# ZhentaoHuang/SealD-NeRF

Measured on AMD Instinct MI355X. Metric: rendered rays/sec + sampled-points/sec, 800×800 D-NeRF jumpingjacks, higher is better.
Workload: dtype f16; 1 GPU; dnerf jumpingjacks-like 800x800 full-frame inference render, -O (fp16 field network, fp16 grid table), test sequence of 20 frames (camera orbit, one time stamp per frame, t = 0 .. 1: every frame selects its own occupancy slice, time encoding and the t == 0 canonical rule), T_thresh 1e-2, max_steps 1024, dt_gamma 0; rays=640000, field=fused, loop=device, frames_per_loop=4, rays_per_loop_on_this_gpu=2560000, frames_in_flight=4 loops of 4 frame(s) (the next starts when the newest is down to rays/2 alive), parallelism=single GPU

## Files before the change

seald-nerf_amd/csrc/raymarching.hip:

```cpp
#include <stdlib.h>

#include "sdn_common.h"
#include "sdn_internal.h"

namespace {
using sdn_int::FrameSel;

constexpr float kSqrt3 = 1.7320508075688772f;
constexpr float kRPi = 0.3183098861837907f;

__device__ __forceinline__ float signf_(float x) { return copysignf(1.0f, x); }
__device__ __forceinline__ float clampf_(float x, float lo, float hi) { return fminf(hi, fmaxf(lo, x)); }

__device__ __forceinline__ int mip_from_pos(float x, float y, float z, float max_cascade) {
    const float mx = fmaxf(fabsf(x), fmaxf(fabsf(y), fabsf(z)));
    int exponent;
    frexpf(mx, &exponent);
    return (int)fminf(max_cascade - 1, fmaxf(0.0f, (float)exponent));
}
__device__ __forceinline__ int mip_from_dt(float dt, float H, float max_cascade) {
    const float mx = (float)((double)(dt * H) * 0.5);
    int exponent;
    frexpf(mx, &exponent);
    return (int)fminf(max_cascade - 1, fmaxf(0.0f, (float)exponent));
// ... 884 lines not shown
__device__ __forceinline__ bool composite_ray(int index, uint32_t n_step, float T_thresh, const float *s, const float *c, const float *dl,
                                              float *__restrict__ rays_t, float *__restrict__ weights_sum, float *__restrict__ depth,
                                              float *__restrict__ image, float *t_out = nullptr) {
    float t = rays_t[index];
    float weight_sum = weights_sum[index], d = depth[index];
    float r = image[(size_t)index * 3], g = image[(size_t)index * 3 + 1], b = image[(size_t)index * 3 + 2];
    uint32_t step = 0;
    if (n_step == 8) {
        float sv[8], cv[24], dv[16];
        #pragma unroll
        for (int q = 0; q < 2; q++) *reinterpret_cast<float4 *>(sv + 4 * q) = *reinterpret_cast<const float4 *>(s + 4 * q);
        #pragma unroll
        for (int q = 0; q < 6; q++) *reinterpret_cast<float4 *>(cv + 4 * q) = *reinterpret_cast<const float4 *>(c + 4 * q);
        #pragma unroll
        for (int q = 0; q < 4; q++) *reinterpret_cast<float4 *>(dv + 4 * q) = *reinterpret_cast<const float4 *>(dl + 4 * q);
        bool open = true;
        #pragma unroll
        for (int k = 0; k < 8; k++) {
            if (open && dv[2 * k] == 0) open = false;
            if (open) {
                const float alpha = 1.0f - sdn_exp_cr(-sv[k] * dv[2 * k]);
                const float T = 1 - weight_sum;
                const float weight = alpha * T;
                weight_sum += weight;
                t += dv[2 * k + 1];
                d += weight * t;
                r += weight * cv[3 * k]; g += weight * cv[3 * k + 1]; b += weight * cv[3 * k + 2];
                if (T < T_thresh) open = false; else step++;
            }
        }
    } else {
        while (step < n_step) {
            if (dl[0] == 0) break;
            const float alpha = 1.0f - sdn_exp_cr(-s[0] * dl[0]);
            const float T = 1 - weight_sum;
            const float weight = alpha * T;
            weight_sum += weight;
            t += dl[1];
            d += weight * t;
            r += weight * c[0]; g += weight * c[1]; b += weight * c[2];
            if (T < T_thresh) break;
            s++; c += 3; dl += 2; step++;
        }
    }
    const bool survives = !(step < n_step);
    if (survives) rays_t[index] = t;
    if (t_out) *t_out = t;
    weights_sum[index] = weight_sum; depth[index] = d;
    image[(size_t)index * 3] = r; image[(size_t)index * 3 + 1] = g; image[(size_t)index * 3 + 2] = b;
    return survives;
}

template <bool FAST>
__global__ void __launch_bounds__(256) k_march_rays(uint32_t n_alive, uint32_t n_step, const int32_t *__restrict__ rays_alive,
                                                    const float *__restrict__ rays_t, const float *__restrict__ rays_o,
                                                    const float *__restrict__ rays_d, float bound, float dt_gamma, uint32_t max_steps,
                                                    uint32_t C, uint32_t H, const uint8_t *__restrict__ grid,
                                                    const float *__restrict__ fars, float *__restrict__ xyzs, float *__restrict__ dirs,
                                                    float *__restrict__ deltas, const float *__restrict__ noises, uint32_t M_pad,
                                                    const uint32_t *__restrict__ cull, uint32_t *__restrict__ live_idx,
                                                    uint32_t *__restrict__ live_count, const int32_t *__restrict__ state,
                                                    const int32_t *__restrict__ rays_alive_b, FrameSel fs, const float *__restrict__ jump) {
    if (state) {
        n_alive = (uint32_t)state[0];
        n_step = (uint32_t)state[1];
        if (n_alive == 0) return;
        if (state[4]) rays_alive = rays_alive_b;
        live_count += state[3];
        const uint32_t m0 = n_alive * n_step;
        M_pad = m0 + (128u - m0 % 128u);
        if (!(state[15] && state[3] == 0)) jump = nullptr;
        if (blockIdx.x * 256u >= n_alive + 128u) return;
    }
    __shared__ uint4 s_cull4[FAST ? 256 : 1];
    __shared__ unsigned long long s_fine[FAST ? kFineCacheCells : 1];
    __shared__ uint32_t s_min4[4];
    const uint32_t n = threadIdx.x + blockIdx.x * blockDim.x;
    const int index = n < n_alive ? rays_alive[n] : -1;
    const bool grouped = fs.n_frames > 1;
    const uint32_t frame = (grouped && index >= 0) ? (uint32_t)index / fs.rays_per_frame : (grouped ? kNoFrame : 0u);
    uint32_t step = 0;
    float ro[3] = {0, 0, 0}, rdv[3] = {0, 0, 1}, t_ray = 0, far_ray = 0, t_jump = 0, noise = 0;
    if (index >= 0) {
        ro[0] = rays_o[(size_t)index * 3]; ro[1] = rays_o[(size_t)index * 3 + 1]; ro[2] = rays_o[(size_t)index * 3 + 2];
        rdv[0] = rays_d[(size_t)index * 3]; rdv[1] = rays_d[(size_t)index * 3 + 1]; rdv[2] = rays_d[(size_t)index * 3 + 2];
        t_ray = rays_t[index]; far_ray = fars[index];
        if (jump) t_jump = jump[index];
        if (noises) noise = noises[n];
    }
    uint32_t fcur = grouped ? block_min_256(frame, s_min4) : 0u;
    while (fcur != kNoFrame) {
        const uint8_t *grid_f = grouped ? frame_grid_uniform(fs, fcur) : grid;
        const uint32_t *cull_f = (grouped && cull) ? cull + (size_t)fcur * fs.cull_stride : cull;
        OccCache oc;
        occ_cache_load<FAST>(cull_f, grid_f, s_cull4, s_fine, oc);
        if (index >= 0 && frame == fcur) {
            MarcherT<FAST> m;
            m.init(ro, rdv, bound, dt_gamma, max_steps, C, H, grid_f);
            float t = t_ray;
            t += m.step_size(t) * noise;
            float *tend = state ? state_tend(state) : nullptr;
            if (tend) tend += index;
            const float t_walk = jump ? t_jump : t;
            step = march_ray<FAST>(m, oc, t_walk, far_ray, n_step, xyzs + (size_t)n * n_step * 3, dirs + (size_t)n * n_step * 3,
                                   deltas + (size_t)n * n_step * 2, tend, grouped ? fs.slot_frame + (size_t)n * n_step : nullptr, frame,
                                   jump ? &t : nullptr);
        }
        if (!grouped) break;
        fcur = block_min_256((frame != kNoFrame && frame > fcur) ? frame : kNoFrame, s_min4);
    }
    if (n >= n_alive) {
        const uint32_t slot = n_alive * n_step + (n - n_alive);
        if (slot < M_pad) {
            xyzs[(size_t)slot * 3] = 0; xyzs[(size_t)slot * 3 + 1] = 0; xyzs[(size_t)slot * 3 + 2] = 0;
            dirs[(size_t)slot * 3] = 0; dirs[(size_t)slot * 3 + 1] = 0; dirs[(size_t)slot * 3 + 2] = 0;
            deltas[(size_t)slot * 2] = 0; deltas[(size_t)slot * 2 + 1] = 0;
        }
    }
    if (live_idx) live_append(step, n, n_step, live_idx, live_count);
}

__device__ __forceinline__ uint32_t loop_list_len(const int32_t *__restrict__ state) {
    return state[8] ? (uint32_t)state[8] : (uint32_t)state[0];
}

__global__ void __launch_bounds__(256) k_composite_rays(uint32_t n_alive, uint32_t n_step, float T_thresh, int32_t *__restrict__ rays_alive,
                                                        float *__restrict__ rays_t, const float *__restrict__ sigmas,
                                                        const float *__restrict__ rgbs, const float *__restrict__ deltas,
                                                        float *__restrict__ weights_sum, float *__restrict__ depth, float *__restrict__ image,
                                                        const int32_t *__restrict__ state, int32_t *__restrict__ rays_alive_b,
                                                        uint32_t *__restrict__ block_totals) {
    if (state) {
        n_alive = loop_list_len(state);
        n_step = (uint32_t)state[1];
        if (state[4]) rays_alive = rays_alive_b;
    }
    const uint32_t n = threadIdx.x + blockIdx.x * blockDim.x;
    bool survives = false;
    if (n < n_alive) {
        const int index = rays_alive[n];
        if (index >= 0) {
            survives = composite_ray(index, n_step, T_thresh, sigmas + (size_t)n * n_step, rgbs + (size_t)n * n_step * 3,
                                     deltas + (size_t)n * n_step * 2, rays_t, weights_sum, depth, image);
            if (!survives) rays_alive[n] = -1;
        }
    }
    if (block_totals) {
        __shared__ uint32_t s_cnt[4];
        const unsigned long long m = __ballot(survives);
        if ((threadIdx.x & 63u) == 0) s_cnt[threadIdx.x >> 6] = (uint32_t)__popcll(m);
        __syncthreads();
        if (threadIdx.x == 0) block_totals[blockIdx.x] = s_cnt[0] + s_cnt[1] + s_cnt[2] + s_cnt[3];
    }
}

__global__ void __launch_bounds__(kScanBlock) k_compact_count(const int32_t *__restrict__ in, uint32_t n, uint32_t *__restrict__ block_totals,
                                                              const int32_t *__restrict__ state, const int32_t *__restrict__ in_b) {
    if (state) {
        n = loop_list_len(state);
        if (state[4]) in = in_b;
        if (blockIdx.x * kScanBlock >= n) return;
    }
    __shared__ uint32_t lds[16];
    const uint32_t i = blockIdx.x * kScanBlock + threadIdx.x;
    const bool keep = i < n && in[i] >= 0;
    const unsigned long long mask = __ballot(keep);
    if ((threadIdx.x & 63u) == 0) lds[threadIdx.x >> 6] = (uint32_t)__popcll(mask);
    __syncthreads();
    if (threadIdx.x == 0) {
        uint32_t t = 0;
        for (uint32_t w = 0; w < (kScanBlock >> 6); w++) t += lds[w];
        block_totals[blockIdx.x] = t;
// ... 332 lines not shown
            if (!survives) alive[n] = -1;
        }
        const bool marches = survives && march_next;
        const bool grouped = fs.n_frames > 1;
        const uint32_t frame = (grouped && marches) ? (uint32_t)index / fs.rays_per_frame : (grouped ? kNoFrame : 0u);
        uint32_t fcur = grouped ? block_min_256(frame, s_min4) : 0u;
        while (fcur != kNoFrame) {
            const uint8_t *grid_f = grouped ? frame_grid_uniform(fs, fcur) : grid;
            const uint32_t *cull_f = (grouped && cull) ? cull + (size_t)fcur * fs.cull_stride : cull;
            OccCache oc;
            occ_cache_load<FAST>(cull_f, grid_f, s_cull4, s_fine, oc);
            if (marches && frame == fcur) {
                float *px = xyzs + (size_t)n * n_step * 3, *pd = dirs + (size_t)n * n_step * 3, *pl = deltas + (size_t)n * n_step * 2;
                MarcherT<FAST> m;
                m.init(ro, rdv, bound, dt_gamma, max_steps, C, H, grid_f);
                float *tend = state_tend(state);
                if (tend) tend += index;
                emitted = march_ray<FAST>(m, oc, t_new, far_ray, n_step, px, pd, pl, tend,
                                          grouped ? fs.slot_frame + (size_t)n * n_step : nullptr, frame);
            }
            if (!grouped) break;
            fcur = block_min_256((frame != kNoFrame && frame > fcur) ? frame : kNoFrame, s_min4);
        }
        live_append(emitted, n, n_step, live_idx, live_counts + it + 1);
    }
    const unsigned long long mask = __ballot(survives);
    if ((threadIdx.x & 63u) == 0) s_cnt[threadIdx.x >> 6] = (uint32_t)__popcll(mask);
    __syncthreads();
    if (threadIdx.x == 0) {
        const uint32_t c = s_cnt[0] + s_cnt[1] + s_cnt[2] + s_cnt[3];
        if (c) atomicAdd(state + 9, (int32_t)c);
        __threadfence();
        s_last = (atomicAdd(ticket, 1) == (int)gridDim.x - 1);
    }
    __syncthreads();
    if (!s_last || threadIdx.x != 0) return;
    __threadfence();
    *ticket = 0;
    const int32_t call = state[7];
    state[7] = call + 1;
    if (state[0] > 0) {
        trace[2 * it] = state[0];
        trace[2 * it + 1] = state[1];
        state[2] += state[1];
        state[3] = it + 1;
        int32_t n_new = atomicAdd(state + 9, 0);
        state[9] = 0;
        if (state[2] >= state[6]) n_new = 0;
        state[0] = n_new;
    }
    publish_snapshot(state, snap, call);
}

__global__ void __launch_bounds__(256) k_loop_finish(uint32_t N, const float *__restrict__ nears, const float *__restrict__ fars,
                                                     const float *__restrict__ weights_sum, const float *__restrict__ depth,
                                                     const float *__restrict__ image, float bg, float *__restrict__ image_out,
                                                     float *__restrict__ depth_out) {
    const uint32_t n = threadIdx.x + blockIdx.x * blockDim.x;
    if (n >= N) return;
    const float w = (1 - weights_sum[n]) * bg;
    image_out[(size_t)n * 3] = image[(size_t)n * 3] + w;
    image_out[(size_t)n * 3 + 1] = image[(size_t)n * 3 + 1] + w;
    image_out[(size_t)n * 3 + 2] = image[(size_t)n * 3 + 2] + w;
    depth_out[n] = fmaxf(depth[n] - nears[n], 0.0f) / (fars[n] - nears[n]);
}

struct MarchRays {
    uint32_t threads = 0;
    uint32_t n_alive = 0, n_step = 0;
    const int32_t *rays_alive = nullptr, *rays_alive_b = nullptr, *state = nullptr;
    const float *rays_t = nullptr, *rays_o = nullptr, *rays_d = nullptr, *fars = nullptr, *noises = nullptr;
    float bound = 0, dt_gamma = 0;
    uint32_t max_steps = 0, C = 0, H = 0, M_pad = 0;
    const uint8_t *grid = nullptr;
    float *xyzs = nullptr, *dirs = nullptr, *deltas = nullptr;
    const uint32_t *cull = nullptr;
    uint32_t *live_idx = nullptr, *live_count = nullptr;
    FrameSel fs;
    const float *jump = nullptr;
};
int launch_k_march_rays(const MarchRays &m, hipStream_t st) {
    const dim3 g(sdn_div_up(m.threads, 256u)), b(256);
    if (fast_config(m.bound, m.C, m.H)) {
        const uint32_t *cull = (m.cull && m.H != 128) ? nullptr : m.cull;
        hipLaunchKernelGGL(k_march_rays<true>, g, b, 0, st, m.n_alive, m.n_step, m.rays_alive, m.rays_t, m.rays_o, m.rays_d, m.bound, m.dt_gamma,
                           m.max_steps, m.C, m.H, m.grid, m.fars, m.xyzs, m.dirs, m.deltas, m.noises, m.M_pad, cull, m.live_idx, m.live_count, m.state,
                           m.rays_alive_b, m.fs, cull ? m.jump : (const float *)nullptr);
    } else {
        hipLaunchKernelGGL(k_march_rays<false>, g, b, 0, st, m.n_alive, m.n_step, m.rays_alive, m.rays_t, m.rays_o, m.rays_d, m.bound, m.dt_gamma,
                           m.max_steps, m.C, m.H, m.grid, m.fars, m.xyzs, m.dirs, m.deltas, m.noises, m.M_pad, (const uint32_t *)nullptr, m.live_idx,
                           m.live_count, m.state, m.rays_alive_b, m.fs, (const float *)nullptr);
    }
    return sdn_launch_status();
}

struct TrainScratch { uint64_t cull, sample_t; };
TrainScratch train_scratch(uint32_t N) {
    const uint64_t words = (uint64_t)N + sdn_div_up(N, kScanBlock) + 4u;
    const uint64_t head = (words * sizeof(uint32_t) + 15u) & ~(uint64_t)15u;
    const uint64_t cull_bytes = ((uint64_t)(kCullWords + 8u) * sizeof(uint32_t) + 15u) & ~(uint64_t)15u;
    return {head, head + cull_bytes};
}

}

namespace sdn_int {

int loop_begin(const SdnRenderCtx &c, void *mailbox, uint32_t frame_tag, hipStream_t st) {
    const uint32_t threads = c.N > c.n_counters ? c.N : c.n_counters;
    hipLaunchKernelGGL(k_loop_init, dim3(sdn_div_up(threads, 256u)), dim3(256), 0, st, c.N, c.max_steps, c.nears, c.alive_a, c.rays_t, c.weights_sum,
                       c.depth, c.image, c.state, c.live_counts, c.n_counters, (unsigned long long)(uintptr_t)mailbox, frame_tag, c.rays_tend);
    return sdn_launch_status();
}

int loop_cull_start(const SdnRenderCtx &c, hipStream_t st) {
    const uint32_t *cull = loop_cull(c);
    if (!cull || !c.rays_tend || c.H != 128 || !fast_config(c.bound, c.C, c.H)) return 0;
    uint32_t *block_totals = (uint32_t *)c.block_totals;
    hipLaunchKernelGGL(k_cull_start, dim3(sdn_div_up(c.N, 256u)), dim3(256), 0, st, c.N, c.rays_o, c.rays_d, c.nears, c.fars, cull, frame_sel(c), c.alive_a,
                       c.rays_tend, c.bound, c.dt_gamma, c.max_steps, c.C, c.H, jump_buffer(c), block_totals);
    const uint32_t nb = sdn_div_up(c.N, kScanBlock);
    hipLaunchKernelGGL(k_compact_scatter, dim3(nb), dim3(kScanBlock), 0, st, (const int32_t *)c.alive_a, c.N, (const uint32_t *)block_totals, c.alive_b,
                       snap_n_out(c), (const int32_t *)nullptr, (const int32_t *)nullptr, (int32_t *)nullptr, 4u);
    hipLaunchKernelGGL(k_cull_advance, dim3(1), dim3(64), 0, st, c.state, (const int32_t *)snap_n_out(c), c.trace);
    return sdn_launch_status();
}

static int march(const SdnRenderCtx &c, uint32_t bound_alive, const float *jump, hipStream_t st) {
    MarchRays m;
    m.threads = bound_alive + 128u;
    m.rays_alive = c.alive_a; m.rays_alive_b = c.alive_b; m.rays_t = c.rays_t; m.rays_o = c.rays_o; m.rays_d = c.rays_d;
    m.bound = c.bound; m.dt_gamma = c.dt_gamma; m.max_steps = c.max_steps; m.C = c.C; m.H = c.H; m.grid = c.bitfield; m.fars = c.fars;
    m.xyzs = c.xyzs; m.dirs = c.dirs; m.deltas = c.deltas; m.cull = loop_cull(c); m.live_idx = c.live_idx; m.live_count = live_counters(c);
    m.state = c.state; m.fs = frame_sel(c); m.jump = jump;
    return launch_k_march_rays(m, st);
}

int loop_march(const SdnRenderCtx &c, uint32_t bound_alive, hipStream_t st) { return march(c, bound_alive, jump_buffer(c), st); }

int loop_composite_compact(const SdnRenderCtx &c, uint32_t bound_alive, hipStream_t st, bool freeze) {
    const dim3 g(sdn_div_up(bound_alive, 256u)), b(256);
    uint32_t *block_totals = (uint32_t *)c.block_totals;
    int32_t *snap = snap_ring(c);
    hipLaunchKernelGGL(k_composite_rays, g, b, 0, st, 0u, 0u, c.T_thresh, c.alive_a, c.rays_t, c.sigmas, c.rgbs, c.deltas, c.weights_sum, c.depth, c.image,
                       (const int32_t *)c.state, c.alive_b, block_totals);
    if (bound_alive > 65536u) {
        static_assert(kScanBlock == 1024, "the compositing kernel's 256-ray survivor counts are summed four to a scatter block");
        const uint32_t nb = sdn_div_up(bound_alive, kScanBlock);
        hipLaunchKernelGGL(k_compact_scatter, dim3(nb), dim3(kScanBlock), 0, st, (const int32_t *)c.alive_a, 0u, (const uint32_t *)block_totals,
                           c.alive_b, snap_n_out(c), (const int32_t *)c.state, (const int32_t *)c.alive_b, c.alive_a, 4u);
        hipLaunchKernelGGL(k_loop_advance, dim3(1), dim3(64), 0, st, c.state, (const int32_t *)snap_n_out(c), c.trace, snap, freeze ? 1 : 0);
        return sdn_launch_status();
    }
    hipLaunchKernelGGL(k_scatter_advance, g, b, 0, st, c.alive_a, c.alive_b, (const uint32_t *)block_totals, c.state, c.n_out, c.trace, snap, freeze ? 1 : 0);
    return sdn_launch_status();
}

int loop_steady_begin(const SdnRenderCtx &c, uint32_t bound_alive, hipStream_t st, bool frozen_already) {
    if (!frozen_already) hipLaunchKernelGGL(k_steady_begin, dim3(1), dim3(64), 0, st, c.state);
    return march(c, bound_alive, nullptr, st);
}

int loop_composite_march(const SdnRenderCtx &c, uint32_t bound_list, hipStream_t st) {
    const dim3 g(sdn_div_up(bound_list, 256u)), b(256);
    const FrameSel fs = frame_sel(c);
    int32_t *snap = snap_ring(c);
    if (fast_config(c.bound, c.C, c.H)) {
        const uint32_t *cull = loop_cull(c);
        if (cull && c.H != 128) cull = nullptr;
        hipLaunchKernelGGL(k_composite_march<true>, g, b, 0, st, c.T_thresh, c.alive_a, c.alive_b, c.rays_t, c.rays_o, c.rays_d, c.bound, c.dt_gamma,
                           c.max_steps, c.C, c.H, c.bitfield, c.fars, c.sigmas, c.rgbs, c.xyzs, c.dirs, c.deltas, c.weights_sum, c.depth, c.image, cull,
                           c.live_idx, live_counters(c), c.state, c.n_out, c.trace, snap, fs);
    } else {
        hipLaunchKernelGGL(k_composite_march<false>, g, b, 0, st, c.T_thresh, c.alive_a, c.alive_b, c.rays_t, c.rays_o, c.rays_d, c.bound, c.dt_gamma,
                           c.max_steps, c.C, c.H, c.bitfield, c.fars, c.sigmas, c.rgbs, c.xyzs, c.dirs, c.deltas, c.weights_sum, c.depth, c.image,
                           (const uint32_t *)nullptr, c.live_idx, live_counters(c), c.state, c.n_out, c.trace, snap, fs);
    }
    return sdn_launch_status();
}

int loop_finish(const SdnRenderCtx &c, float bg, float *image_out, float *depth_out, hipStream_t st) {
    hipLaunchKernelGGL(k_loop_finish, dim3(sdn_div_up(c.N, 256u)), dim3(256), 0, st, c.N, c.nears, c.fars, c.weights_sum, c.depth, c.image, bg, image_out,
                       depth_out);
    return sdn_launch_status();
}

int build_cull(const uint8_t *bitfield, uint32_t *cull_bits, hipStream_t st, bool with_image) {
    hipLaunchKernelGGL(k_cull_meta_init, dim3(1), dim3(64), 0, st, cull_bits, 1u, 0u);
    hipLaunchKernelGGL(k_build_cull_grid, dim3(kCullRes * kCullRes * kCullRes / 256), dim3(256), 0, st, bitfield, cull_bits, FrameSel());
    if (with_image) hipLaunchKernelGGL(k_build_fine_image, dim3(kFineCacheCells / 256), dim3(256), 0, st, bitfield, cull_bits, FrameSel());
    return sdn_launch_status();
}

struct CullCopy { const uint32_t *src[SDN_MAX_GROUP_FRAMES]; };
__global__ void __launch_bounds__(256) k_copy_cull_grids(CullCopy srcs, uint32_t *__restrict__ dst, uint32_t words, uint32_t stride) {
    const uint32_t i = blockIdx.x * blockDim.x + threadIdx.x;
    if (i < words) dst[(size_t)blockIdx.y * stride + i] = srcs.src[blockIdx.y][i];
}

int copy_cull(const void *const *prebuilt, uint32_t n_frames, uint32_t *cull_bits, hipStream_t st) {
    CullCopy c{};
    for (uint32_t f = 0; f < n_frames && f < (uint32_t)SDN_MAX_GROUP_FRAMES; f++) c.src[f] = (const uint32_t *)prebuilt[f];
    const uint32_t words = sdn_cull_grid_bytes() / 4u;
    hipLaunchKernelGGL(k_copy_cull_grids, dim3(sdn_div_up(words, 256u), n_frames), dim3(256), 0, st, c, cull_bits, words, n_frames > 1 ? words : 0u);
    return sdn_launch_status();
}

int build_cull_group(const FrameSel &fs, uint32_t *cull_bits, hipStream_t st) {
    hipLaunchKernelGGL(k_cull_meta_init, dim3(1), dim3(64), 0, st, cull_bits, fs.n_frames, fs.cull_stride);
    hipLaunchKernelGGL(k_build_cull_grid, dim3(kCullRes * kCullRes * kCullRes / 256, fs.n_frames), dim3(256), 0, st, (const uint8_t *)nullptr,
// ... 229 lines not shown
```

seald-nerf_amd/csrc/render.hip:

```cpp
#include <atomic>
#include <chrono>
#include <stdio.h>
#include <stdlib.h>
#include <string.h>

#include "sdn_common.h"
#include "sdn_internal.h"

namespace sdn_int {
int render_begin(const SdnRenderCtx *c, void *mailbox, uint32_t frame_tag, hipStream_t st) {
    if (c->aabb) {
        int rc0 = sdn_near_far_from_aabb(c->rays_o, c->rays_d, c->aabb, c->N, c->min_near, (float *)c->nears, (float *)c->fars, st);
        if (rc0) return rc0;
    }
    int rc = loop_begin(*c, mailbox, frame_tag, st);
    if (rc) return rc;
    if (has_loop_cull(*c)) {
        const uint32_t nf = c->n_group_frames > 1 ? c->n_group_frames : 1u;
        bool kept = true;
        for (uint32_t f = 0; f < nf; f++) kept = kept && c->frame_cull[f] != nullptr;
        if (kept) rc = copy_cull(c->frame_cull, nf, (uint32_t *)c->cull_bits, st);
        else rc = c->n_group_frames > 1 ? build_cull_group(frame_sel(*c), (uint32_t *)c->cull_bits, st) : build_cull(c->bitfield, (uint32_t *)c->cull_bits, st);
        if (!rc && c->rays_tend) rc = loop_cull_start(*c, st);
    }
    return rc;
}
}

namespace {
std::atomic<int> g_timed_kernel{0};
}

extern "C" {

int sdn_render_time_kernel(int which) {
    if (which < 0 || which > 1) return SDN_E_BADARG;
    g_timed_kernel.store(which);
    return 0;
}

static int seal_map(const SdnRenderCtx &c, uint32_t m_slots, hipStream_t st) {
    const SdnSealBox *s = c.seal;
    if (!s) return 0;
    if (!c.seal_mask) return SDN_E_BADARG;
    if (s->has_map_source) {
        if (!s->scratch) return SDN_E_BADARG;
        return sdn_seal_bbox_map_source(c.xyzs, c.dirs, m_slots, s->bounds, s->n_bounds, s->tris, s->n_tris, s->test_dir, s->tinv, s->rinv,
                                        s->scale, s->center, s->source_bound, s->map_source, (uint32_t *)((char *)s->scratch + 16), c.seal_mask,
                                        c.live_idx, sdn_int::live_counters(c), c.state, st);
    }
    return sdn_seal_bbox_map(c.xyzs, c.dirs, m_slots, s->bounds, s->n_bounds, s->tris, s->n_tris, s->test_dir, s->tinv, s->rinv, s->scale,
                             s->center, c.seal_mask, st);
}
static int seal_color(const SdnRenderCtx &c, uint32_t m_slots, hipStream_t st) {
    const SdnSealBox *s = c.seal;
    if (!s) return 0;
    int rc = 0;
    if (s->modify_hsv) rc = sdn_seal_modify_hsv(c.rgbs, c.seal_mask, m_slots, s->hsv[0], s->hsv[1], s->hsv[2], st);
    if (!rc && s->modify_rgb) {
        if (!s->scratch) return SDN_E_BADARG;
        rc = sdn_seal_modify_rgb(c.rgbs, c.seal_mask, m_slots, s->rgb[0], s->rgb[1], s->rgb[2], s->rgb_light_offset, s->scratch, c.live_idx,
                                 sdn_int::live_counters(c), c.state, st);
    }
    return rc;
}

static int launch_field(const SdnRenderCtx &c, uint32_t m_bound, uint32_t expect_points, hipStream_t st) {
    const bool group = c.n_group_frames > 1;
    return sdn_int::field_forward(c.field_f32,
                                  {.xyzs = c.xyzs, .dirs = c.dirs, .live_idx = c.live_idx, .live_count = sdn_int::live_counters(c), .state = c.state,
                                   .M = m_bound, .weights = c.field_weights, .bias0 = c.field_bias0, .table = c.grid_table,
                                   .offsets_host = c.grid_offsets, .S = c.grid_S, .H = c.grid_H, .bound = c.bound,
                                   .density_scale = c.density_scale, .zero_deform = c.zero_deform, .sigmas = c.sigmas, .rgbs = c.rgbs,
                                   .expect_points = expect_points, .slot_frame = group ? c.slot_frame : nullptr,
                                   .n_frames = group ? c.n_group_frames : 1u},
                                  st);
}
// ... 31 lines not shown
    int rc = sdn_int::loop_march(*c, bound_alive, st);
    if (time_march && ev_field_end) (void)hipEventRecord((hipEvent_t)ev_field_end, st);
    if (time_march) ev_field_begin = ev_field_end = nullptr;
    if (rc) return rc;
    uint64_t m_bound = (uint64_t)bound_alive * 8u;
    if (m_bound > c->N) m_bound = c->N;
    rc = seal_map(*c, (uint32_t)m_bound, st);
    if (rc) return rc;
    if (ev_field_begin) (void)hipEventRecord((hipEvent_t)ev_field_begin, st);
    rc = launch_field(*c, (uint32_t)m_bound, 0u, st);
    if (ev_field_end) (void)hipEventRecord((hipEvent_t)ev_field_end, st);
    if (rc) return rc;
    rc = seal_color(*c, (uint32_t)m_bound, st);
    if (rc) return rc;
    return sdn_int::loop_composite_compact(*c, bound_alive, st);
}

}

namespace {

constexpr uint32_t kRecompactMin = 8192;
uint32_t recompact_pct(uint32_t list_len) { return list_len > 81920u ? 95u : 50u; }
constexpr int kDriverTimeoutSeconds = 20;

struct FrameRun {
    const SdnRenderCtx *c;
    hipStream_t st, side;
    void **ev_main, **ev_copy, **ev_field;
    int32_t *host_snap;
    uint32_t max_field_events;
    uint32_t bound, it;
    bool steady, done;
    bool recompact = false;
    uint32_t list_bound = 0;
    void *mail_dev = nullptr;
    uint32_t tag = 0;
    uint32_t last_alive = 0;

    int begin() {
        if (!ctx_ok(c)) return SDN_E_BADARG;
        bound = c->N; it = 0; steady = false; done = false; last_alive = c->N; recompact = false; list_bound = 0;
        mail_dev = nullptr;
        unsigned int flags = 0;
        void *dptr = nullptr;
        if (hipHostGetFlags(&flags, host_snap) == hipSuccess && (flags & hipHostMallocCoherent) &&
            hipHostGetDevicePointer(&dptr, host_snap, 0) == hipSuccess && dptr) {
            static std::atomic<uint32_t> frame_seq{0};
            tag = (frame_seq.fetch_add(1) % 0x7FFFu) + 1u;
            mail_dev = dptr;
        } else {
            (void)hipGetLastError();
        }
        return sdn_int::render_begin(c, mail_dev, tag, st);
    }

    int enqueue() {
        void *e0 = (ev_field && it < max_field_events) ? ev_field[2 * it] : nullptr;
        void *e1 = (ev_field && it < max_field_events) ? ev_field[2 * it + 1] : nullptr;
        int rc;
        if (!steady) {
            rc = sdn_render_step_f16_ev(c, bound, e0, e1, st);
        } else {
            uint64_t m_bound = (uint64_t)bound * 8u;
            if (m_bound > c->N) m_bound = c->N;
            rc = seal_map(*c, (uint32_t)m_bound, st);
            if (rc) return rc;
            const bool time_march = g_timed_kernel.load() == 1;
            void *m0 = time_march ? e0 : nullptr, *m1 = time_march ? e1 : nullptr;
            if (time_march) e0 = e1 = nullptr;
            if (e0) (void)hipEventRecord((hipEvent_t)e0, st);
            rc = launch_field(*c, (uint32_t)m_bound, last_alive * 8u, st);
            if (e1) (void)hipEventRecord((hipEvent_t)e1, st);
            if (!rc) rc = seal_color(*c, (uint32_t)m_bound, st);
            if (!rc && m0) (void)hipEventRecord((hipEvent_t)m0, st);
            if (!rc && recompact) {
                rc = sdn_int::loop_composite_compact(*c, bound, st, true);
                const uint32_t nb = last_alive < bound ? last_alive : bound;
                if (!rc) rc = sdn_int::loop_steady_begin(*c, nb, st, true);
                bound = list_bound = nb;
                recompact = false;
            } else if (!rc)
                rc = sdn_int::loop_composite_march(*c, bound, st);
            if (!rc && m1) (void)hipEventRecord((hipEvent_t)m1, st);
        }
        if (rc) return rc;
        if (mail_dev) return 0;
        const uint32_t slot = it & 3u;
        hipError_t e = hipEventRecord((hipEvent_t)ev_main[slot], st);
        if (e == hipSuccess) e = hipStreamWaitEvent(side, (hipEvent_t)ev_main[slot], 0);
        if (e == hipSuccess) e = hipMemcpyAsync(host_snap + 2 * slot, sdn_int::snap_ring(*c) + 2 * slot, 2 * sizeof(int32_t), hipMemcpyDeviceToHost, side);
        if (e == hipSuccess) e = hipEventRecord((hipEvent_t)ev_copy[slot], side);
        return (int)e;
    }

    bool ready() const {
        if (it == 0) return true;
        const uint32_t prev = (it - 1) & 3u;
        if (mail_dev) {
            const uint64_t want = ((uint64_t)tag << 16) | it;
            return (__atomic_load_n(reinterpret_cast<const uint64_t *>(host_snap) + prev, __ATOMIC_ACQUIRE) >> 32) == want;
        }
        return hipEventQuery((hipEvent_t)ev_copy[prev]) == hipSuccess;
    }

    int settle() {
        if (it >= 1) {
            const uint32_t prev = (it - 1) & 3u;
            int32_t n_prev;
            if (mail_dev) {
                const uint64_t want = ((uint64_t)tag << 16) | it;
                const uint64_t *word = reinterpret_cast<const uint64_t *>(host_snap) + prev;
                uint64_t v;
                uint32_t spins = 0;
                auto t0 = std::chrono::steady_clock::now();
                auto t_query = t0;
                while (((v = __atomic_load_n(word, __ATOMIC_ACQUIRE)) >> 32) != want) {
                    if ((++spins & 0x3FFFu) == 0) {
                        const auto now = std::chrono::steady_clock::now();
                        if (now - t0 > std::chrono::seconds(kDriverTimeoutSeconds)) return SDN_E_TIMEOUT;
                        if (now - t_query > std::chrono::milliseconds(5)) {
                            t_query = now;
                            hipError_t q = hipStreamQuery(st);
                            if (q != hipSuccess && q != hipErrorNotReady) return (int)q;
                        }
                    }
                }
                n_prev = (int32_t)(uint32_t)v;
            } else {
                hipError_t e = hipEventSynchronize((hipEvent_t)ev_copy[prev]);
                if (e != hipSuccess) return (int)e;
                n_prev = host_snap[2 * prev];
            }
            if (n_prev <= 0) { done = true; return 0; }
            last_alive = (uint32_t)n_prev;
            if (!steady) {
                bound = (uint32_t)n_prev;
                if ((uint64_t)n_prev * 8u <= c->N) {
                    int rc = sdn_int::loop_steady_begin(*c, bound, st);
                    if (rc) return rc;
                    steady = true;
                    list_bound = bound;
                }
            } else if ((uint64_t)n_prev * 100u <= (uint64_t)list_bound * recompact_pct(list_bound) && (uint32_t)n_prev >= kRecompactMin) {
                recompact = true;
            }
        }
        it++;
        if (it > c->max_steps + 1) done = true;
        return 0;
    }
};

}

extern "C" {

int sdn_render_frame_f16(const SdnRenderCtx *c, float bg_color, float *image_out, float *depth_out, void *stream, void *side_stream,
                         void **ev_main, void **ev_copy, int32_t *host_snap, void **ev_field, uint32_t max_field_events,
                         uint32_t *iterations_out) {
    if (!c || !image_out || !depth_out || !side_stream || !ev_main || !ev_copy || !host_snap) return SDN_E_BADARG;
    FrameRun r{c, (hipStream_t)stream, (hipStream_t)side_stream, ev_main, ev_copy, ev_field, host_snap, max_field_events, 0, 0, false, false};
    int rc = r.begin();
    while (!rc && !r.done) {
        rc = r.enqueue();
        if (!rc) rc = r.settle();
    }
    if (rc) return rc;
    if (iterations_out) *iterations_out = r.it + 1;
    return sdn_render_finish(c, bg_color, image_out, depth_out, stream);
}

int sdn_render_frames_pipelined_f16(const SdnRenderCtx *const *ctxs, uint32_t n_ctx, uint32_t n_frames, const float *const *rays_o,
                                    const float *const *rays_d, float *const *image_outs, float *const *depth_outs, float bg_color,
                                    uint32_t overlap_div, void *const *streams, void *const *side_streams, void **ev_main, void **ev_copy,
                                    int32_t *host_snap, void *const *ev_field_frames, uint32_t max_field_events, const uint8_t *exclusive_frames,
                                    const SdnFrameTime *frame_times, void *const *done_events, uint32_t *iterations_out) {
    constexpr uint32_t kMaxCtx = 8;
    if (!ctxs || n_ctx == 0 || n_ctx > kMaxCtx || !rays_o || !rays_d || !image_outs || !depth_outs || !streams || !side_streams ||
        !ev_main || !ev_copy || !host_snap)
        return SDN_E_BADARG;
    for (uint32_t s = 0; s < n_ctx; s++)
        if (!ctxs[s] || !ctxs[s]->aabb || !side_streams[s]) return SDN_E_BADARG;
    if (n_frames == 0) return 0;
    if (overlap_div == 0) overlap_div = 1;
    SdnRenderCtx local[kMaxCtx];
    FrameRun runs[kMaxCtx];
    int frame_of[kMaxCtx];
    for (uint32_t s = 0; s < n_ctx; s++) { local[s] = *ctxs[s]; frame_of[s] = -1; }
    uint32_t next = 0, finished = 0;
    auto start = [&](uint32_t slot) -> int {
        if (!rays_o[next] || !rays_d[next] || !image_outs[next] || !depth_outs[next]) return SDN_E_BADARG;
// ... 126 lines not shown
```

seald-nerf_amd/csrc/sdn_internal.h:

```cpp
#pragma once
#include "sdn_common.h"

namespace sdn_int {

struct FrameSel {
    uint32_t n_frames = 0;
    uint32_t rays_per_frame = 0;
    uint32_t cull_stride = 0;
    uint32_t pad_ = 0;
    const uint8_t *grid[SDN_MAX_GROUP_FRAMES] = {};
    uint8_t *slot_frame = nullptr;
};
FrameSel frame_sel(const SdnRenderCtx &c);

inline int32_t *snap_ring(const SdnRenderCtx &c) { return c.trace + 2 * (size_t)c.n_counters; }
inline int32_t *snap_n_out(const SdnRenderCtx &c) { return snap_ring(c) + 8; }
inline uint32_t *live_counters(const SdnRenderCtx &c) { return (uint32_t *)c.live_counts; }
inline float *jump_buffer(const SdnRenderCtx &c) { return c.rays_tend ? c.sigmas : nullptr; }
inline bool has_loop_cull(const SdnRenderCtx &c) { return c.H == 128 && c.C == 1; }
inline const uint32_t *loop_cull(const SdnRenderCtx &c) { return has_loop_cull(c) ? (const uint32_t *)c.cull_bits : nullptr; }

int loop_begin(const SdnRenderCtx &c, void *mailbox, uint32_t frame_tag, hipStream_t st);
int loop_cull_start(const SdnRenderCtx &c, hipStream_t st);
int loop_march(const SdnRenderCtx &c, uint32_t bound_alive, hipStream_t st);
int loop_composite_compact(const SdnRenderCtx &c, uint32_t bound_alive, hipStream_t st, bool freeze = false);
int loop_steady_begin(const SdnRenderCtx &c, uint32_t bound_alive, hipStream_t st, bool frozen_already = false);
int loop_composite_march(const SdnRenderCtx &c, uint32_t bound_list, hipStream_t st);
int loop_finish(const SdnRenderCtx &c, float bg, float *image_out, float *depth_out, hipStream_t st);
int render_begin(const SdnRenderCtx *c, void *mailbox, uint32_t frame_tag, hipStream_t st);
int build_cull(const uint8_t *bitfield, uint32_t *cull_bits, hipStream_t st, bool with_image = true);
int march_rays_train(const float *rays_o, const float *rays_d, const uint8_t *grid, float bound, float dt_gamma, uint32_t max_steps, uint32_t N, uint32_t C,
                     uint32_t H, uint32_t M, const float *nears, const float *fars, float *xyzs, float *dirs, float *deltas, int32_t *rays, int32_t *counter,
                     const float *noises, void *scratch, const void *prebuilt_cull, hipStream_t st);
int build_cull_group(const FrameSel &fs, uint32_t *cull_bits, hipStream_t st);
int copy_cull(const void *const *prebuilt, uint32_t n_frames, uint32_t *cull_bits, hipStream_t st);

struct FieldCall {
    const float *xyzs = nullptr, *dirs = nullptr;
    const uint32_t *live_idx = nullptr, *live_count = nullptr;
    const int32_t *state = nullptr;
    uint32_t M = 0;
    const void *weights = nullptr;
    const float *bias0 = nullptr;
    const void *table = nullptr;
    const int32_t *offsets_host = nullptr;
    float S = 0;
    uint32_t H = 0;
    float bound = 0, density_scale = 0;
    int zero_deform = 0;
    float *sigmas = nullptr, *rgbs = nullptr;
    float *deform = nullptr;
    uint32_t expect_points = 0;
    const uint8_t *slot_frame = nullptr;
    uint32_t n_frames = 1;
};
struct FieldCells {
    FieldCall f;
    const float *noise = nullptr;
    uint32_t seed = 0, grid_size = 0;
    float cas_bound = 0;
};

inline uint32_t field_n_frames(const FieldCall &f) {
    if (!f.slot_frame || f.n_frames == 0) return 1u;
    return f.n_frames > (uint32_t)SDN_MAX_GROUP_FRAMES ? (uint32_t)SDN_MAX_GROUP_FRAMES : f.n_frames;
}

int field_forward_f16(const FieldCall &f, hipStream_t st);
int field_forward_f32(const FieldCall &f, hipStream_t st);
int field_forward_f32x3(const FieldCall &f, hipStream_t st);
int field_cells_f16(const FieldCells &q, hipStream_t st);
int field_cells_f32(const FieldCells &q, hipStream_t st);
inline int field_forward(int kind, const FieldCall &f, hipStream_t st) {
    return kind == 2 ? field_forward_f32x3(f, st) : (kind ? field_forward_f32(f, st) : field_forward_f16(f, st));
}

inline bool field_buffers_ok(const FieldCall &f) {
    if (!f.weights || !f.bias0 || !f.table || !f.offsets_host || !f.sigmas) return false;
    if ((f.live_idx == nullptr) != (f.live_count == nullptr)) return false;
    return ((uintptr_t)f.weights & 15u) == 0 && ((uintptr_t)f.table & 3u) == 0;
}
inline int field_forward_checked(int kind, const FieldCall &f, void *stream) {
// ... 27 lines not shown
```

Measured before the change: 3.219 billion sampled-points/s.

## Fuse alive-list compaction with ray marching into a single kernel

Adds a k_compact_march kernel that scans the per-block alive totals, gathers the surviving ray indices in order and marches them in the same launch, using a last-block ticket to update the loop state. The non-steady loop iterations and the start of a render now use this fused compact+march path instead of separate compact, state-update and march launches. The marching body is factored into a shared device function. This removes kernel launches and a round trip of the alive list through global memory, at the cost of a heavier kernel with more shared memory, a redundant per-block scan of the block totals, and more complex state bookkeeping.

New measurement: 2.116 billion sampled-points/s. 34.3% lower.

```diff
diff --git a/seald-nerf_amd/csrc/raymarching.hip b/seald-nerf_amd/csrc/raymarching.hip
--- a/seald-nerf_amd/csrc/raymarching.hip
+++ b/seald-nerf_amd/csrc/raymarching.hip
@@ -960,6 +960,57 @@
 }
 
 template <bool FAST>
+__device__ __forceinline__ void march_block(int index, uint32_t n, uint32_t n_alive, uint32_t n_step, const float *__restrict__ rays_t,
+                                            const float *__restrict__ rays_o, const float *__restrict__ rays_d, float bound, float dt_gamma,
+                                            uint32_t max_steps, uint32_t C, uint32_t H, const uint8_t *__restrict__ grid,
+                                            const float *__restrict__ fars, float *__restrict__ xyzs, float *__restrict__ dirs,
+                                            float *__restrict__ deltas, const float *__restrict__ noises, uint32_t M_pad,
+                                            const uint32_t *__restrict__ cull, uint32_t *__restrict__ live_idx,
+                                            uint32_t *__restrict__ live_count, float *__restrict__ tend_base, const FrameSel &fs,
+                                            const float *__restrict__ jump, uint4 *s_cull4, unsigned long long *s_fine, uint32_t *s_min4) {
+    const bool grouped = fs.n_frames > 1;
+    const uint32_t frame = (grouped && index >= 0) ? (uint32_t)index / fs.rays_per_frame : (grouped ? kNoFrame : 0u);
+    uint32_t step = 0;
+    float ro[3] = {0, 0, 0}, rdv[3] = {0, 0, 1}, t_ray = 0, far_ray = 0, t_jump = 0, noise = 0;
+    if (index >= 0) {
+        ro[0] = rays_o[(size_t)index * 3]; ro[1] = rays_o[(size_t)index * 3 + 1]; ro[2] = rays_o[(size_t)index * 3 + 2];
+        rdv[0] = rays_d[(size_t)index * 3]; rdv[1] = rays_d[(size_t)index * 3 + 1]; rdv[2] = rays_d[(size_t)index * 3 + 2];
+        t_ray = rays_t[index]; far_ray = fars[index];
+        if (jump) t_jump = jump[index];
+        if (noises) noise = noises[n];
+    }
+    uint32_t fcur = grouped ? block_min_256(frame, s_min4) : 0u;
+    while (fcur != kNoFrame) {
+        const uint8_t *grid_f = grouped ? frame_grid_uniform(fs, fcur) : grid;
+        const uint32_t *cull_f = (grouped && cull) ? cull + (size_t)fcur * fs.cull_stride : cull;
+        OccCache oc;
+        occ_cache_load<FAST>(cull_f, grid_f, s_cull4, s_fine, oc);
+        if (index >= 0 && frame == fcur) {
+            MarcherT<FAST> m;
+            m.init(ro, rdv, bound, dt_gamma, max_steps, C, H, grid_f);
+            float t = t_ray;
+            t += m.step_size(t) * noise;
+            float *tend = tend_base ? tend_base + index : nullptr;
+            const float t_walk = jump ? t_jump : t;
+            step = march_ray<FAST>(m, oc, t_walk, far_ray, n_step, xyzs + (size_t)n * n_step * 3, dirs + (size_t)n * n_step * 3,
+                                   deltas + (size_t)n * n_step * 2, tend, grouped ? fs.slot_frame + (size_t)n * n_step : nullptr, frame,
+                                   jump ? &t : nullptr);
+        }
+        if (!grouped) break;
+        fcur = block_min_256((frame != kNoFrame && frame > fcur) ? frame : kNoFrame, s_min4);
+    }
+    if (n >= n_alive) {
+        const uint32_t slot = n_alive * n_step + (n - n_alive);
+        if (slot < M_pad) {
+            xyzs[(size_t)slot * 3] = 0; xyzs[(size_t)slot * 3 + 1] = 0; xyzs[(size_t)slot * 3 + 2] = 0;
+            dirs[(size_t)slot * 3] = 0; dirs[(size_t)slot * 3 + 1] = 0; dirs[(size_t)slot * 3 + 2] = 0;
+            deltas[(size_t)slot * 2] = 0; deltas[(size_t)slot * 2 + 1] = 0;
+        }
+    }
+    if (live_idx) live_append(step, n, n_step, live_idx, live_count);
+}
+
+template <bool FAST>
 __global__ void __launch_bounds__(256) k_march_rays(uint32_t n_alive, uint32_t n_step, const int32_t *__restrict__ rays_alive,
                                                     const float *__restrict__ rays_t, const float *__restrict__ rays_o,
                                                     const float *__restrict__ rays_d, float bound, float dt_gamma, uint32_t max_steps,
@@ -985,47 +1036,8 @@
     __shared__ uint32_t s_min4[4];
     const uint32_t n = threadIdx.x + blockIdx.x * blockDim.x;
     const int index = n < n_alive ? rays_alive[n] : -1;
-    const bool grouped = fs.n_frames > 1;
-    const uint32_t frame = (grouped && index >= 0) ? (uint32_t)index / fs.rays_per_frame : (grouped ? kNoFrame : 0u);
-    uint32_t step = 0;
-    float ro[3] = {0, 0, 0}, rdv[3] = {0, 0, 1}, t_ray = 0, far_ray = 0, t_jump = 0, noise = 0;
-    if (index >= 0) {
-        ro[0] = rays_o[(size_t)index * 3]; ro[1] = rays_o[(size_t)index * 3 + 1]; ro[2] = rays_o[(size_t)index * 3 + 2];
-        rdv[0] = rays_d[(size_t)index * 3]; rdv[1] = rays_d[(size_t)index * 3 + 1]; rdv[2] = rays_d[(size_t)index * 3 + 2];
-        t_ray = rays_t[index]; far_ray = fars[index];
-        if (jump) t_jump = jump[index];
-        if (noises) noise = noises[n];
-    }
-    uint32_t fcur = grouped ? block_min_256(frame, s_min4) : 0u;
-    while (fcur != kNoFrame) {
-        const uint8_t *grid_f = grouped ? frame_grid_uniform(fs, fcur) : grid;
-        const uint32_t *cull_f = (grouped && cull) ? cull + (size_t)fcur * fs.cull_stride : cull;
-        OccCache oc;
-        occ_cache_load<FAST>(cull_f, grid_f, s_cull4, s_fine, oc);
-        if (index >= 0 && frame == fcur) {
-            MarcherT<FAST> m;
-            m.init(ro, rdv, bound, dt_gamma, max_steps, C, H, grid_f);
-            float t = t_ray;
-            t += m.step_size(t) * noise;
-            float *tend = state ? state_tend(state) : nullptr;
-            if (tend) tend += index;
-            const float t_walk = jump ? t_jump : t;
-            step = march_ray<FAST>(m, oc, t_walk, far_ray, n_step, xyzs + (size_t)n * n_step * 3, dirs + (size_t)n * n_step * 3,
-                                   deltas + (size_t)n * n_step * 2, tend, grouped ? fs.slot_frame + (size_t)n * n_step : nullptr, frame,
-                                   jump ? &t : nullptr);
-        }
-        if (!grouped) break;
-        fcur = block_min_256((frame != kNoFrame && frame > fcur) ? frame : kNoFrame, s_min4);
-    }
-    if (n >= n_alive) {
-        const uint32_t slot = n_alive * n_step + (n - n_alive);
-        if (slot < M_pad) {
-            xyzs[(size_t)slot * 3] = 0; xyzs[(size_t)slot * 3 + 1] = 0; xyzs[(size_t)slot * 3 + 2] = 0;
-            dirs[(size_t)slot * 3] = 0; dirs[(size_t)slot * 3 + 1] = 0; dirs[(size_t)slot * 3 + 2] = 0;
-            deltas[(size_t)slot * 2] = 0; deltas[(size_t)slot * 2 + 1] = 0;
-        }
-    }
-    if (live_idx) live_append(step, n, n_step, live_idx, live_count);
+    march_block<FAST>(index, n, n_alive, n_step, rays_t, rays_o, rays_d, bound, dt_gamma, max_steps, C, H, grid, fars, xyzs, dirs, deltas, noises,
+                      M_pad, cull, live_idx, live_count, state ? state_tend(state) : nullptr, fs, jump, s_cull4, s_fine, s_min4);
 }
 
 __device__ __forceinline__ uint32_t loop_list_len(const int32_t *__restrict__ state) {
@@ -1464,6 +1476,142 @@
     publish_snapshot(state, snap, call);
 }
 
+template <bool FAST>
+__global__ void __launch_bounds__(256) k_compact_march(uint32_t start_n, int32_t *__restrict__ alive_a, int32_t *__restrict__ alive_b,
+                                                       const uint32_t *__restrict__ block_totals, const float *__restrict__ rays_t,
+                                                       const float *__restrict__ rays_o, const float *__restrict__ rays_d, float bound,
+                                                       float dt_gamma, uint32_t max_steps, uint32_t C, uint32_t H,
+                                                       const uint8_t *__restrict__ grid, const float *__restrict__ fars,
+                                                       float *__restrict__ xyzs, float *__restrict__ dirs, float *__restrict__ deltas,
+                                                       const uint32_t *__restrict__ cull, uint32_t *__restrict__ live_idx,
+                                                       uint32_t *__restrict__ live_counts, int32_t *__restrict__ state,
+                                                       int32_t *__restrict__ ticket, int32_t *__restrict__ trace, int32_t *__restrict__ snap,
+                                                       FrameSel fs, const float *__restrict__ jump, int freeze) {
+    __shared__ uint4 s_cull4[FAST ? 256 : 1];
+    __shared__ unsigned long long s_fine[FAST ? kFineCacheCells : 1];
+    __shared__ uint32_t s_min4[4], s_scan[16], s_wc[16], s_find[2];
+    __shared__ int32_t s_out[256];
+    __shared__ int s_last;
+    const bool start = start_n != 0;
+    const int32_t n_old = state[0], n_step_old = state[1], steps_done = state[2], it = state[3], N = state[5], steps_max = state[6];
+    const bool side = !start && state[4];
+    const uint32_t list_len = start ? start_n : loop_list_len(state);
+    float *tend_base = state_tend(state);
+    const int32_t *__restrict__ in = side ? alive_b : alive_a;
+    int32_t *__restrict__ out = side ? alive_a : alive_b;
+    const uint32_t n = threadIdx.x + blockIdx.x * 256u;
+    uint32_t total = 0;
+    if (n_old > 0) {
+        const uint32_t nb_in = (list_len + 255u) / 256u;
+        const uint32_t chunk = (nb_in + 255u) / 256u;
+        const uint32_t b0 = min(threadIdx.x * chunk, nb_in), b1 = min(b0 + chunk, nb_in);
+        uint32_t part = 0;
+        for (uint32_t b = b0; b < b1; b++) part += block_totals[b];
+        const uint32_t incl = block_inclusive_scan(part, s_scan, total);
+        const uint32_t out0 = blockIdx.x * 256u;
+        int index = -1;
+        if (out0 < total) {
+            if (incl - part <= out0 && out0 < incl) {
+                uint32_t cum = incl - part, j = b0;
+                while (j + 1 < b1) {
+                    const uint32_t c = block_totals[j];
+                    if (cum + c > out0) break;
+                    cum += c; j++;
+                }
+                s_find[0] = j; s_find[1] = cum;
+            }
+            __syncthreads();
+            uint32_t j = s_find[0], cum = s_find[1];
+            const uint32_t out1 = min(out0 + 256u, total);
+            const uint32_t lane = threadIdx.x & 63u, wid = threadIdx.x >> 6;
+            while (cum < out1 && j < nb_in) {
+                int32_t v[4];
+                uint32_t below[4];
+                #pragma unroll
+                for (uint32_t q = 0; q < 4; q++) {
+                    const uint32_t i = (j + q) * 256u + threadIdx.x;
+                    v[q] = i < list_len ? in[i] : -1;
+                }
+                #pragma unroll
+                for (uint32_t q = 0; q < 4; q++) {
+                    const unsigned long long mask = __ballot(v[q] >= 0);
+                    below[q] = (uint32_t)__popcll(mask & ((1ull << lane) - 1ull));
+                    if (lane == 0) s_wc[q * 4u + wid] = (uint32_t)__popcll(mask);
+                }
+                __syncthreads();
+                uint32_t pre = cum, base[4] = {0, 0, 0, 0};
+                #pragma unroll
+                for (uint32_t k = 0; k < 16; k++) {
+                    if ((k & 3u) == wid) base[k >> 2] = pre;
+                    pre += s_wc[k];
+                }
+                #pragma unroll
+                for (uint32_t q = 0; q < 4; q++) {
+                    const uint32_t r = base[q] + below[q] - out0;
+                    if (v[q] >= 0 && r < 256u) s_out[r] = v[q];
+                }
+                cum = pre; j += 4u;
+                __syncthreads();
+            }
+            if (n < total) { index = s_out[threadIdx.x]; out[n] = index; }
+        }
+        uint32_t n_new = total, n_step_new = (uint32_t)n_step_old;
+        uint32_t *live_count = live_counts + it;
+        if (!start) {
+            if (steps_done + n_step_old >= steps_max) n_new = 0;
+            if (n_new > 0) { const uint32_t ns = (uint32_t)N / n_new; n_step_new = ns > 8u ? 8u : (ns < 1u ? 1u : ns); }
+            live_count++;
+            jump = nullptr;
+        }
+        if (n_new > 0 && blockIdx.x * 256u < n_new + 128u) {
+            const uint32_t m0 = n_new * n_step_new;
+            march_block<FAST>(index, n, n_new, n_step_new, rays_t, rays_o, rays_d, bound, dt_gamma, max_steps, C, H, grid, fars, xyzs, dirs, deltas,
+                              nullptr, m0 + (128u - m0 % 128u), cull, live_idx, live_count, tend_base, fs, jump, s_cull4, s_fine, s_min4);
+        }
+    }
+    __syncthreads();
+    if (threadIdx.x == 0) {
+        __threadfence();
+        s_last = (atomicAdd(ticket, 1) == (int)gridDim.x - 1);
+    }
+    __syncthreads();
+    if (!s_last || threadIdx.x != 0) return;
+    __threadfence();
+    *ticket = 0;
+    if (start) {
+        state[4] = 1;
+        state[15] = 1;
+        if (total > 0) {
+            state[0] = (int32_t)total;
+        } else {
+            trace[0] = N;
+            trace[1] = n_step_old;
+            state[2] = steps_done + n_step_old;
+            state[3] = 1;
+            state[0] = 0;
+        }
+        return;
+    }
+    const int32_t call = state[7];
+    state[7] = call + 1;
+    if (n_old > 0) {
+        trace[2 * it] = (it == 0 && state[15]) ? N : n_old;
+        trace[2 * it + 1] = n_step_old;
+        state[2] = steps_done + n_step_old;
+        state[3] = it + 1;
+        state[4] ^= 1;
+        int32_t n_new = (int32_t)total;
+        if (steps_done + n_step_old >= steps_max) n_new = 0;
+        state[0] = n_new;
+        if (n_new > 0) {
+            const int32_t ns = N / n_new;
+            state[1] = ns > 8 ? 8 : (ns < 1 ? 1 : ns);
+        }
+    }
+    if (freeze) { state[8] = state[0]; state[9] = 0; }
+    publish_snapshot(state, snap, call);
+}
+
 __global__ void __launch_bounds__(256) k_loop_finish(uint32_t N, const float *__restrict__ nears, const float *__restrict__ fars,
                                                      const float *__restrict__ weights_sum, const float *__restrict__ depth,
                                                      const float *__restrict__ image, float bg, float *__restrict__ image_out,
@@ -1568,6 +1716,46 @@
     return sdn_launch_status();
 }
 
+static int compact_march(const SdnRenderCtx &c, uint32_t start_n, uint32_t bound_new, bool freeze, hipStream_t st) {
+    if (bound_new > c.N) bound_new = c.N;
+    const dim3 g(sdn_div_up(bound_new + 128u, 256u)), b(256);
+    const FrameSel fs = frame_sel(c);
+    const uint32_t *block_totals = (const uint32_t *)c.block_totals;
+    int32_t *snap = snap_ring(c);
+    if (fast_config(c.bound, c.C, c.H)) {
+        const uint32_t *cull = loop_cull(c);
+        if (cull && c.H != 128) cull = nullptr;
+        hipLaunchKernelGGL(k_compact_march<true>, g, b, 0, st, start_n, c.alive_a, c.alive_b, block_totals, (const float *)c.rays_t, c.rays_o, c.rays_d,
+                           c.bound, c.dt_gamma, c.max_steps, c.C, c.H, c.bitfield, c.fars, c.xyzs, c.dirs, c.deltas, cull, c.live_idx, live_counters(c),
+                           c.state, c.n_out, c.trace, snap, fs, cull ? (const float *)jump_buffer(c) : (const float *)nullptr, freeze ? 1 : 0);
+    } else {
+        hipLaunchKernelGGL(k_compact_march<false>, g, b, 0, st, start_n, c.alive_a, c.alive_b, block_totals, (const float *)c.rays_t, c.rays_o, c.rays_d,
+                           c.bound, c.dt_gamma, c.max_steps, c.C, c.H, c.bitfield, c.fars, c.xyzs, c.dirs, c.deltas, (const uint32_t *)nullptr, c.live_idx,
+                           live_counters(c), c.state, c.n_out, c.trace, snap, fs, (const float *)nullptr, freeze ? 1 : 0);
+    }
+    return sdn_launch_status();
+}
+
+bool loop_has_cull_start(const SdnRenderCtx &c) { return loop_cull(c) && c.rays_tend && c.H == 128 && fast_config(c.bound, c.C, c.H); }
+
+int loop_cull_start_march(const SdnRenderCtx &c, hipStream_t st) {
+    if (!loop_has_cull_start(c)) return SDN_E_BADARG;
+    hipLaunchKernelGGL(k_cull_start, dim3(sdn_div_up(c.N, 256u)), dim3(256), 0, st, c.N, c.rays_o, c.rays_d, c.nears, c.fars, loop_cull(c), frame_sel(c),
+                       c.alive_a, c.rays_tend, c.bound, c.dt_gamma, c.max_steps, c.C, c.H, jump_buffer(c), (uint32_t *)c.block_totals);
+    return compact_march(c, c.N, c.N, false, st);
+}
+
+int loop_composite_compact_march(const SdnRenderCtx &c, uint32_t bound_list, uint32_t bound_new, hipStream_t st, bool freeze) {
+    hipLaunchKernelGGL(k_composite_rays, dim3(sdn_div_up(bound_list, 256u)), dim3(256), 0, st, 0u, 0u, c.T_thresh, c.alive_a, c.rays_t, c.sigmas, c.rgbs,
+                       c.deltas, c.weights_sum, c.depth, c.image, (const int32_t *)c.state, c.alive_b, (uint32_t *)c.block_totals);
+    return compact_march(c, 0u, bound_new, freeze, st);
+}
+
+int loop_freeze(const SdnRenderCtx &c, hipStream_t st) {
+    hipLaunchKernelGGL(k_steady_begin, dim3(1), dim3(64), 0, st, c.state);
+    return sdn_launch_status();
+}
+
 int loop_steady_begin(const SdnRenderCtx &c, uint32_t bound_alive, hipStream_t st, bool frozen_already) {
     if (!frozen_already) hipLaunchKernelGGL(k_steady_begin, dim3(1), dim3(64), 0, st, c.state);
     return march(c, bound_alive, nullptr, st);
diff --git a/seald-nerf_amd/csrc/render.hip b/seald-nerf_amd/csrc/render.hip
--- a/seald-nerf_amd/csrc/render.hip
+++ b/seald-nerf_amd/csrc/render.hip
@@ -8,7 +8,7 @@
 #include "sdn_internal.h"
 
 namespace sdn_int {
-int render_begin(const SdnRenderCtx *c, void *mailbox, uint32_t frame_tag, hipStream_t st) {
+int render_begin(const SdnRenderCtx *c, void *mailbox, uint32_t frame_tag, hipStream_t st, bool march_first) {
     if (c->aabb) {
         int rc0 = sdn_near_far_from_aabb(c->rays_o, c->rays_d, c->aabb, c->N, c->min_near, (float *)c->nears, (float *)c->fars, st);
         if (rc0) return rc0;
@@ -21,8 +21,10 @@
         for (uint32_t f = 0; f < nf; f++) kept = kept && c->frame_cull[f] != nullptr;
         if (kept) rc = copy_cull(c->frame_cull, nf, (uint32_t *)c->cull_bits, st);
         else rc = c->n_group_frames > 1 ? build_cull_group(frame_sel(*c), (uint32_t *)c->cull_bits, st) : build_cull(c->bitfield, (uint32_t *)c->cull_bits, st);
+        if (!rc && march_first && loop_has_cull_start(*c)) return loop_cull_start_march(*c, st);
         if (!rc && c->rays_tend) rc = loop_cull_start(*c, st);
     }
+    if (!rc && march_first) rc = loop_march(*c, c->N, st);
     return rc;
 }
 }
@@ -160,38 +162,34 @@
         } else {
             (void)hipGetLastError();
         }
-        return sdn_int::render_begin(c, mail_dev, tag, st);
+        return sdn_int::render_begin(c, mail_dev, tag, st, true);
     }
 
     int enqueue() {
         void *e0 = (ev_field && it < max_field_events) ? ev_field[2 * it] : nullptr;
         void *e1 = (ev_field && it < max_field_events) ? ev_field[2 * it + 1] : nullptr;
-        int rc;
-        if (!steady) {
-            rc = sdn_render_step_f16_ev(c, bound, e0, e1, st);
-        } else {
-            uint64_t m_bound = (uint64_t)bound * 8u;
-            if (m_bound > c->N) m_bound = c->N;
-            rc = seal_map(*c, (uint32_t)m_bound, st);
-            if (rc) return rc;
-            const bool time_march = g_timed_kernel.load() == 1;
-            void *m0 = time_march ? e0 : nullptr, *m1 = time_march ? e1 : nullptr;
-            if (time_march) e0 = e1 = nullptr;
-            if (e0) (void)hipEventRecord((hipEvent_t)e0, st);
-            rc = launch_field(*c, (uint32_t)m_bound, last_alive * 8u, st);
-            if (e1) (void)hipEventRecord((hipEvent_t)e1, st);
-            if (!rc) rc = seal_color(*c, (uint32_t)m_bound, st);
-            if (!rc && m0) (void)hipEventRecord((hipEvent_t)m0, st);
-            if (!rc && recompact) {
-                rc = sdn_int::loop_composite_compact(*c, bound, st, true);
-                const uint32_t nb = last_alive < bound ? last_alive : bound;
-                if (!rc) rc = sdn_int::loop_steady_begin(*c, nb, st, true);
-                bound = list_bound = nb;
-                recompact = false;
-            } else if (!rc)
-                rc = sdn_int::loop_composite_march(*c, bound, st);
-            if (!rc && m1) (void)hipEventRecord((hipEvent_t)m1, st);
-        }
+        uint64_t m_bound = (uint64_t)bound * 8u;
+        if (m_bound > c->N) m_bound = c->N;
+        int rc = seal_map(*c, (uint32_t)m_bound, st);
+        if (rc) return rc;
+        const bool time_march = g_timed_kernel.load() == 1;
+        void *m0 = time_march ? e0 : nullptr, *m1 = time_march ? e1 : nullptr;
+        if (time_march) e0 = e1 = nullptr;
+        if (e0) (void)hipEventRecord((hipEvent_t)e0, st);
+        rc = launch_field(*c, (uint32_t)m_bound, steady ? last_alive * 8u : 0u, st);
+        if (e1) (void)hipEventRecord((hipEvent_t)e1, st);
+        if (!rc) rc = seal_color(*c, (uint32_t)m_bound, st);
+        if (!rc && m0) (void)hipEventRecord((hipEvent_t)m0, st);
+        if (!rc && !steady) {
+            rc = sdn_int::loop_composite_compact_march(*c, bound, last_alive < bound ? last_alive : bound, st);
+        } else if (!rc && recompact) {
+            const uint32_t nb = last_alive < bound ? last_alive : bound;
+            rc = sdn_int::loop_composite_compact_march(*c, bound, nb, st, true);
+            bound = list_bound = nb;
+            recompact = false;
+        } else if (!rc)
+            rc = sdn_int::loop_composite_march(*c, bound, st);
+        if (!rc && m1) (void)hipEventRecord((hipEvent_t)m1, st);
         if (rc) return rc;
         if (mail_dev) return 0;
         const uint32_t slot = it & 3u;
@@ -245,7 +243,7 @@
             if (!steady) {
                 bound = (uint32_t)n_prev;
                 if ((uint64_t)n_prev * 8u <= c->N) {
-                    int rc = sdn_int::loop_steady_begin(*c, bound, st);
+                    int rc = sdn_int::loop_freeze(*c, st);
                     if (rc) return rc;
                     steady = true;
                     list_bound = bound;
diff --git a/seald-nerf_amd/csrc/sdn_internal.h b/seald-nerf_amd/csrc/sdn_internal.h
--- a/seald-nerf_amd/csrc/sdn_internal.h
+++ b/seald-nerf_amd/csrc/sdn_internal.h
@@ -26,8 +26,12 @@
 int loop_composite_compact(const SdnRenderCtx &c, uint32_t bound_alive, hipStream_t st, bool freeze = false);
 int loop_steady_begin(const SdnRenderCtx &c, uint32_t bound_alive, hipStream_t st, bool frozen_already = false);
 int loop_composite_march(const SdnRenderCtx &c, uint32_t bound_list, hipStream_t st);
+bool loop_has_cull_start(const SdnRenderCtx &c);
+int loop_cull_start_march(const SdnRenderCtx &c, hipStream_t st);
+int loop_composite_compact_march(const SdnRenderCtx &c, uint32_t bound_list, uint32_t bound_new, hipStream_t st, bool freeze = false);
+int loop_freeze(const SdnRenderCtx &c, hipStream_t st);
 int loop_finish(const SdnRenderCtx &c, float bg, float *image_out, float *depth_out, hipStream_t st);
-int render_begin(const SdnRenderCtx *c, void *mailbox, uint32_t frame_tag, hipStream_t st);
+int render_begin(const SdnRenderCtx *c, void *mailbox, uint32_t frame_tag, hipStream_t st, bool march_first = false);
 int build_cull(const uint8_t *bitfield, uint32_t *cull_bits, hipStream_t st, bool with_image = true);
 int march_rays_train(const float *rays_o, const float *rays_d, const uint8_t *grid, float bound, float dt_gamma, uint32_t max_steps, uint32_t N, uint32_t C,
                      uint32_t H, uint32_t M, const float *nears, const float *fars, float *xyzs, float *dirs, float *deltas, int32_t *rays, int32_t *counter,
```
